# DCDmllm/AnyEdit

Hardware: AMD Instinct MI355X
Metric: edited-images/sec @512x512, 50 DDIM steps (higher is better)
Workload: dtype bf16; 1 GPU; configs[1]: AnySD (SD-1.5 UNet in=8 + task embedding/expert adapters) 512x512 bf16, 50 DDIM steps, batch=4/GPU, 3-branch CFG (UNet batch 12); images_per_gpu=4, ddim_steps=50, cfg_branches=3, hip_graph=True, parallelism=dp1 (image-sharded, no data-path collective)

## Files before the change

anyedit_amd/_lib.py:

```python
import ctypes
import os

import torch

_HERE = os.path.dirname(os.path.abspath(__file__))
LIB_PATH = os.environ.get("AE_LIB_PATH") or os.path.join(_HERE, "libanyedit_hip.so")

c_void_p, c_int, c_long, c_float = ctypes.c_void_p, ctypes.c_int, ctypes.c_long, ctypes.c_float

SIGNATURES = {
    "ae_version": [],
    "ae_last_error": [],
    "ae_device_arch": [ctypes.c_char_p, c_int],
    "ae_device_info": [ctypes.POINTER(c_int), ctypes.POINTER(c_long), ctypes.POINTER(c_int)],
    "ae_gemm_bf16": [c_void_p, c_long, c_void_p, c_long, c_int, c_void_p, c_long, c_void_p, c_long, c_int, c_int, c_int,
                     c_void_p, c_void_p, c_long, c_void_p, c_long, c_int, c_int, c_int, c_void_p, c_void_p],
    "ae_conv3x3_workspace_floats": [c_int, c_int, c_int, c_int, c_int, c_int, c_int],
    "ae_conv3x3_partials_bf16": [c_void_p, c_void_p, c_int, c_int, c_int, c_int, c_int, c_void_p, c_int, c_void_p, c_void_p],
    "ae_groupnorm_splitk_supported": [c_int, c_int, c_int, c_int, c_int],
    "ae_groupnorm_splitk_nhwc_bf16": [c_void_p, c_int, c_void_p, c_void_p, c_long, c_void_p, c_void_p, c_void_p, c_int, c_int, c_int, c_int, c_float, c_int, c_void_p],
    "ae_conv3x3_bf16": [c_void_p, c_void_p, c_void_p, c_void_p, c_long, c_void_p, c_void_p, c_int, c_int, c_int, c_int, c_int,
                        c_int, c_int, c_int, c_void_p, c_void_p, c_int, c_void_p],
    "ae_conv3x3_up2_bf16": [c_void_p, c_void_p, c_void_p, c_void_p, c_int, c_int, c_int, c_int, c_int, c_void_p, c_void_p],
    "ae_groupnorm_rows_per_chunk": [c_int, c_int],
# ... 16 lines not shown
    "ae_add_bf16": [c_void_p, c_void_p, c_void_p, c_long, c_void_p],
    "ae_axpy_bf16": [c_void_p, c_void_p, c_float, c_void_p, c_long, c_void_p],
    "ae_geglu_fwd_bf16": [c_void_p, c_void_p, c_long, c_int, c_void_p],
    "ae_geglu_bwd_bf16": [c_void_p, c_void_p, c_void_p, c_long, c_int, c_void_p],
    "ae_sumpool2x2_bf16": [c_void_p, c_void_p, c_int, c_int, c_int, c_int, c_void_p],
    "ae_colsum_bf16_f32": [c_void_p, c_void_p, c_int, c_int, c_long, c_void_p],
    "ae_mse_grad_f32": [c_void_p, c_void_p, c_void_p, c_long, c_float, c_void_p],
    "ae_adamw_f32": [c_void_p, c_void_p, c_void_p, c_void_p, c_long, c_float, c_float, c_float, c_float, c_float, c_int, c_float,
                     c_void_p],
    "ae_rowsum_f32": [c_void_p, c_void_p, c_int, c_long, c_void_p],
    "ae_scatter_add_rows_f32": [c_void_p, c_void_p, c_void_p, c_int, c_int, c_int, c_void_p],
    "ae_attn_fp8_workspace_bytes": [c_int, c_int, c_int, c_int, c_int],
    "ae_attn_fwd_fp8": [c_void_p, c_void_p, c_void_p, c_void_p, c_int, c_int, c_int, c_int, c_int] + [c_long] * 12 +
                       [c_float, c_void_p, c_void_p, c_int, c_int, c_void_p, c_long, c_void_p],
    "ae_ln_gemm_supported": [c_int, c_int, c_int, c_int],
    "ae_ln_gemm_bf16": [c_void_p, c_long, c_void_p, c_long, c_void_p, c_long, c_int, c_int, c_int, c_void_p, c_void_p, c_long, c_void_p, c_void_p,
                        c_float, c_int, c_void_p, c_void_p],
    "ae_gemm_ln_plan": [c_int, c_int, c_int, c_int, c_int],
    "ae_xattn_fused_supported": [c_int, c_int, c_int, c_int, c_int, c_int, c_int],
    "ae_xattn_fused_covers": [c_int, c_int, c_int, c_int, c_int, c_int, c_int],
    "ae_xattn_fused_kv_bytes": [],
    "ae_xattn_fused_bf16": [c_void_p, c_long, c_void_p, c_void_p, c_float, c_void_p, c_void_p, c_void_p, c_void_p, c_void_p, c_void_p, c_long, c_int, c_int, c_int, c_int,
                            c_float, c_void_p],
    "ae_ff_fused_supported": [c_int, c_int, c_int],
    "ae_ff_fused_bf16": [c_void_p, c_long, c_void_p, c_void_p, c_float, c_void_p, c_long, c_void_p, c_void_p, c_void_p, c_void_p, c_long,
                         c_void_p, c_long, c_void_p, c_void_p, c_long, c_void_p, c_void_p, c_long, c_int, c_int, c_int, c_void_p],
    "ae_gemm_ln_bf16": [c_void_p, c_long, c_void_p, c_long, c_void_p, c_long, c_int, c_int, c_int, c_void_p, c_void_p, c_long, c_int, c_void_p,
                        c_void_p, c_int, c_void_p, c_float, c_void_p],
    "ae_task_gate_bwd": [c_void_p, c_void_p, c_void_p, c_void_p, c_int, c_int, c_int, c_void_p, c_void_p],
    "ae_task_gate_wgrad": [c_void_p, c_void_p, c_void_p, c_void_p, c_void_p, c_int, c_int, c_int, c_int, c_void_p, c_void_p, c_void_p],
    "ae_expert_kv_fwd": [c_void_p, c_void_p, c_void_p, c_void_p, c_int, c_int, c_int, c_int, c_int, c_void_p],
    "ae_expert_kv_dgrad_slices": [c_int],
    "ae_expert_kv_dgrad": [c_void_p, c_void_p, c_void_p, c_void_p, c_int, c_int, c_int, c_int, c_int, c_void_p, c_void_p],
    "ae_expert_kv_wgrad": [c_void_p, c_void_p, c_void_p, c_void_p, c_int, c_int, c_int, c_int, c_int, c_void_p],
    "ae_transpose_last2": [c_void_p, c_void_p, c_int, c_int, c_int, c_int, c_int, c_int, c_void_p],
    "ae_concat_channels_bf16": [c_void_p, c_int, c_void_p, c_int, c_void_p, c_long, c_void_p],
    "ae_im2col3x3_c8_bf16": [c_void_p, c_void_p, c_int, c_int, c_int, c_void_p],
    "ae_split_channels_bf16": [c_void_p, c_int, c_int, c_void_p, c_void_p, c_long, c_int, c_int, c_void_p],
    "ae_timestep_embedding": [c_void_p, c_void_p, c_void_p, c_void_p, c_int, c_int, c_float, c_void_p],
    "ae_ddim_step_f32": [c_void_p, c_void_p, c_void_p, c_void_p, c_void_p, c_void_p, c_long, c_int, c_float, c_float, c_float,
                         c_float, c_float, c_float, c_float, c_float, c_void_p],
    "ae_ddim_encode_step_f32": [c_void_p, c_void_p, c_void_p, c_long, c_int, c_float, c_float, c_float, c_void_p],
    "ae_plms_combine_f32": [c_void_p, c_void_p, c_void_p, c_void_p, c_void_p, c_long, c_int, c_void_p],
    "ae_mask_blend_f32": [c_void_p, c_void_p, c_void_p, c_void_p, c_void_p, c_int, c_int, c_int, c_float, c_float, c_int, c_void_p],
    "ae_q_sample_f32": [c_void_p, c_void_p, c_void_p, c_void_p, c_void_p, c_int, c_long, c_void_p],
    "ae_silu_to_bf16": [c_void_p, c_int, c_void_p, c_long, c_void_p],
# ... 69 lines not shown
```

anyedit_amd/anysd/model.py:

```python
import torch
import torch.nn as nn

from anyedit_amd import ops
from anyedit_amd.cldm.model import trusted_torch_load
from anyedit_amd.ldm.modules.attention import BasicTransformerBlock

BF16 = torch.bfloat16

EDIT_TYPES = ["add", "remove", "replace", "color_alter", "appearance_alter", "material_alter", "action_change",
              "textual_change", "background_change", "tone_transfer", "style_change", "movement", "outpaint", "rotation_change",
              "resize", "implicit_change", "relation_change", "counting", "visual_reference", "visual_bbox", "visual_depth",
              "visual_scribble", "visual_segment", "visual_sketch", "visual_material_transfer"]


class ImageProjModel(nn.Module):

    def __init__(self, clip_dim=1280, cross_dim=768, tokens=4):
        super().__init__()
        self.tokens, self.cross_dim = tokens, cross_dim
        self.proj = nn.Linear(clip_dim, tokens * cross_dim)
        self.norm = nn.LayerNorm(cross_dim)

    def rows(self, ref_embeds):
        B = ref_embeds.shape[0]
# ... 34 lines not shown
    @torch.no_grad()
    def prepare_conditioning(self, encoder_hidden_states, ref_embeds, edit_code, ip_scale=None):
        B, L, Dc = encoder_hidden_states.shape
        dev = encoder_hidden_states.device
        te = self.task_embs.detach()[edit_code.long()]
        ctx = torch.cat([encoder_hidden_states.float(), te[:, None, :].float()], dim=1)
        context_rows = ctx.reshape(B * (L + 1), Dc).to(BF16).contiguous()
        probs, top1, top1p = self.route(edit_code)
        gate = top1p if ip_scale is None else top1p * ip_scale
        ip_rows = self.image_proj_model.rows(ref_embeds)
        T_ip = self.image_proj_model.tokens
        kv_cache = {}
        for blk, W in zip(self._blocks, self.adapter_modules):
            attn = blk.attn2
            kv_cache[id(attn)] = attn.project_kv(context_rows)
            Wm = W.detach()
            if Wm.dtype != torch.float32 or not Wm.is_contiguous():
                Wm = Wm.float().contiguous()
            kv_ip = ops.expert_kv(ip_rows, Wm, top1, T_ip)
            kv_cache[("adapter", id(attn))] = (kv_ip, gate.float().contiguous())
            img = attn.fused_kv_images(kv_cache[id(attn)], kv_cache[("adapter", id(attn))], B)
            if img is not None:
                kv_cache[("xattn_img", id(attn))] = img
        return context_rows, kv_cache

    @torch.no_grad()
    def denoise(self, x, timesteps, context_rows, kv_cache, emb_pack=None):
        return self.unet.forward_rows(x, timesteps, context_rows, kv_cache=kv_cache, emb_pack=emb_pack)

    def forward(self, noisy_latents, timesteps, encoder_hidden_states, image_embeds, edit_code):
        context_rows, kv_cache = self.prepare_conditioning(encoder_hidden_states, image_embeds, edit_code)
        return self.denoise(noisy_latents, timesteps, context_rows, kv_cache)
```

anyedit_amd/build.py:

```python
import hashlib
import os
import shutil
import subprocess
import sys

HERE = os.path.dirname(os.path.abspath(__file__))
CSRC = os.path.join(HERE, "csrc")
LIB = os.path.join(HERE, "libanyedit_hip.so")
SOURCES = ["c_api.hip", "gemm_conv.hip", "gemm_rowpanel.hip", "ff_fused.hip", "xattn_fused.hip", "attention.hip", "attention_fast.hip", "attention_fp8.hip", "attention_bwd.hip", "norm.hip", "elementwise.hip", "backward.hip", "gate.hip", "expert_kv.hip", "msda.hip",
           "sam_decoder.hip", "clip_text.hip"]
EXTRA = {"gemm_conv.hip": ["-fno-slp-vectorize"], "gemm_rowpanel.hip": ["-fno-slp-vectorize"], "ff_fused.hip": ["-fno-slp-vectorize"], "xattn_fused.hip": ["-fno-slp-vectorize"], "attention.hip": ["-ffinite-math-only"],
         "attention_fast.hip": ["-ffinite-math-only", "-fno-slp-vectorize"], "attention_fp8.hip": ["-ffinite-math-only"],
         "attention_bwd.hip": ["-ffinite-math-only"], "clip_text.hip": ["-ffinite-math-only"]}
FLAGS = ["--offload-arch=gfx950", "-O3", "-std=c++17", "-fPIC", "-fno-gpu-rdc", "-Wno-unused-result"]


def _hipcc():
    for c in (shutil.which("hipcc"), "/opt/rocm/bin/hipcc"):
        if c and os.path.exists(c):
            return c
    raise RuntimeError("hipcc not found: the HIP extension cannot be built")


def _digest():
    h = hashlib.sha256()
    for name in sorted(os.listdir(CSRC)):
        with open(os.path.join(CSRC, name), "rb") as f:
            h.update(name.encode() + f.read())
    h.update((" ".join(FLAGS) + repr(sorted(EXTRA.items()))).encode())
    return h.hexdigest()


def build_library(force=False, verbose=True, variant=None, extra_flags=None):
    lib = LIB if variant is None else os.path.join(HERE, f"libanyedit_hip_{variant}.so")
    extra = {k: list(v) for k, v in EXTRA.items()}
# ... 47 lines not shown
```

anyedit_amd/ldm/modules/attention.py:

```python
import os

import torch
import torch.nn as nn

from anyedit_amd import ops
from anyedit_amd.ldm.util import default, exists
from anyedit_amd.ldm.modules.diffusionmodules.util import Linear, Conv2d, LayerNorm, checkpoint

BF16 = torch.bfloat16
_XATTN_FUSED = os.environ.get("AE_XATTN_FUSED", "0") != "0"
_FF_TAIL = os.environ.get("AE_FF_TAIL", "1") != "0"
_SEG2_160 = os.environ.get("AE_ATTN_SEG2_160", "1") != "0"


def zero_module(module):
    for p in module.parameters():
        p.detach().zero_()
    return module


class _GN6(nn.GroupNorm):

    def _affine(self):
        if ops.cache_stale(self, "_pk", self.weight, self.bias):
# ... 133 lines not shown
                pk["qkv"] = torch.cat([wq, wk, wv], 0).contiguous()
            self._pk = pk
        return self._pk

    def _packed_x(self):
        if ops.cache_stale(self, "_pkx", self.to_q.weight, self.to_out[0].weight, self.to_out[0].bias):
            bo = self.to_out[0].bias
            self._pkx = (ops.pack_xattn_wq(self.to_q.weight), ops.pack_xattn_wo(self.to_out[0].weight), None if bo is None else bo.detach().float().contiguous())
        return self._pkx

    def fused_kv_images(self, kv, adapter, B):
        if not _XATTN_FUSED or self.is_self or self.heads != 8 or self.dim_head != 40 or self.to_q.weight.shape[1] != 320:
            return None
        Nk = kv.shape[0] // B
        T = 0 if adapter is None else adapter[0].shape[0] // B
        if not (64 < Nk <= 80 and T <= 16):
            return None
        return ops.pack_xattn_kv(kv, None if adapter is None else adapter[0], B, Nk, T)

    def project_kv(self, ctx_rows):
        return ops.gemm(ctx_rows, self._packed()["kv"])

    def rows(self, x, B, N, context_rows=None, Nk=None, kv=None, key_mask=None, residual=None, adapter=None, norm=None, rowstats=None,
             out_rowstats=None, kv_img=None):
        h, d = self.heads, self.dim_head
        inner = h * d
        if kv_img is not None and kv is not None and norm is not None and residual is x and key_mask is None and out_rowstats is None:
            Nk_ = kv.shape[0] // B
            T_ = 0 if adapter is None else adapter[0].shape[0] // B
            if ops.xattn_fused_ok(x.shape[0], x.shape[1], h, d, N, Nk_, T_):
                wq_img, wo_img, bo = self._packed_x()
                g_, be_ = norm._affine()
                return ops.xattn_fused(x, g_, be_, norm.eps, wq_img, kv_img, None if adapter is None else adapter[1], wo_img, bo, N, Nk_, T_, self.scale)
        pk = self._packed()

        def proj(wname):
            if norm is None:
                return ops.gemm(x, pk[wname])
            if rowstats is not None and ops.ln_fold_plan(x.shape[0], pk[wname].shape[0], x.shape[1], ops.EPI_NONE, 2):
                wq, s, c = self._packed_ln(wname, norm)
                return ops.gemm_ln(x, rowstats, wq, s, c, norm.eps)
            g, be = norm._affine()
            return ops.ln_gemm(x, g, be, norm.eps, pk[wname])

        if context_rows is None and kv is None:
            qkv = proj("qkv")
            s = (N * 3 * inner, d, 3 * inner)
            o = ops.attention(qkv, qkv[:, inner:], qkv[:, 2 * inner:], B, h, N, N, d, self.scale, s, s, s, key_mask=key_mask)
        else:
            q = proj("q")
            if kv is None:
                kv = self.project_kv(context_rows)
            Nk = kv.shape[0] // B
            qs = (N * inner, d, inner)
            ks = (Nk * 2 * inner, d, 2 * inner)
            if adapter is not None and (d <= 96 or (d == 160 and _SEG2_160)) and key_mask is None:
                kv_ip, gate = adapter
                T_ip = kv_ip.shape[0] // B
                ks_ip = (T_ip * 2 * inner, d, 2 * inner)
                seg2 = (kv_ip, kv_ip[:, inner:], T_ip, ks_ip, ks_ip, gate)
                o = ops.attention(q, kv, kv[:, inner:], B, h, N, Nk, d, self.scale, qs, ks, ks, seg2=seg2)
            else:
                o = ops.attention(q, kv, kv[:, inner:], B, h, N, Nk, d, self.scale, qs, ks, ks, key_mask=key_mask)
                if adapter is not None:
                    kv_ip, gate = adapter
                    T_ip = kv_ip.shape[0] // B
                    ks_ip = (T_ip * 2 * inner, d, 2 * inner)
                    ops.attention(q, kv_ip, kv_ip[:, inner:], B, h, N, T_ip, d, self.scale, qs, ks_ip, ks_ip, out=o,
                                  out_scale=gate, accumulate=True)
        return self.to_out[0].rows(o.reshape(B * N, inner), residual=residual, rowstats=out_rowstats)

    def forward(self, x, context=None, mask=None):
        B, N, C = x.shape
        xr = x.reshape(B * N, C).to(BF16).contiguous()
        ctx = None
        if context is not None:
            ctx = context.reshape(-1, context.shape[-1]).to(BF16).contiguous()
        km = None
        if exists(mask):
# ... 59 lines not shown
        M, C = x.shape
        f1, f2, f3 = self._fold_plan(M, C)
        kv2, adapter, kv_img = None, None, None
        if kv_cache is not None and context_rows is not None and not (ops._TAPE is not None and ops._TAPE.active):
            kv_img = kv_cache.get(("xattn_img", id(self.attn2)))
        use_x = kv_img is not None and not f3 and ops.xattn_fused_ok(M, C, self.attn2.heads, self.attn2.dim_head, N, 78, 0)
        st2 = ops.rowstats_buffer(M, C, x.device) if (f2 and not use_x) else None
        st3 = ops.rowstats_buffer(M, C, x.device) if f3 else None
        x = self.attn1.rows(x, B, N, context_rows=c1, residual=x, norm=self.norm1, rowstats=rowstats if f1 else None, out_rowstats=st2)
        if kv_cache is not None and context_rows is not None:
            key = id(self.attn2)
            kv2 = kv_cache.get(key)
            if kv2 is None:
                kv2 = self.attn2.project_kv(context_rows)
                if not (ops._TAPE is not None and ops._TAPE.active):
                    kv_cache[key] = kv2
            adapter = kv_cache.get(("adapter", key))
            if callable(adapter):
                adapter = adapter()
            if kv_img is None and not f3 and not (ops._TAPE is not None and ops._TAPE.active):
                img = self.attn2.fused_kv_images(kv2, adapter, B)
                if img is not None:
                    kv_cache[("xattn_img", key)] = img
        x = self.attn2.rows(x, B, N, context_rows=context_rows, kv=kv2, residual=x, adapter=adapter, norm=self.norm2, rowstats=st2, out_rowstats=st3,
                            kv_img=kv_img if use_x else None)
        x = self.ff.rows(x, residual=x, norm=self.norm3, rowstats=st3, tail=tail)
        return x

    def forward(self, x, context=None):
        B, N, C = x.shape
        ctx = None if context is None else context.reshape(-1, context.shape[-1]).to(BF16).contiguous()
        y = self.rows(x.reshape(B * N, C).to(BF16).contiguous(), B, N, context_rows=ctx)
        return y.reshape(B, N, C).to(x.dtype)

    _forward = forward


class SpatialTransformer(nn.Module):

    def __init__(self, in_channels, n_heads, d_head, depth=1, dropout=0., context_dim=None, disable_self_attn=False,
                 use_linear=False, use_checkpoint=True):
        super().__init__()
        if exists(context_dim) and not isinstance(context_dim, list):
            context_dim = [context_dim] * depth
        if context_dim is None:
            context_dim = [None] * depth
        self.in_channels = in_channels
        inner_dim = n_heads * d_head
# ... 46 lines not shown
```

anyedit_amd/ops.py:

```python
import torch

import ctypes
import os
import threading

from ._lib import lib, check as _check

BF16 = torch.bfloat16
EPI_NONE, EPI_GELU, EPI_GEGLU, EPI_SILU, EPI_RELU = 0, 1, 2, 3, 4


def _s():
    return torch.cuda.current_stream().cuda_stream


def _p(t):
    return None if t is None else t.data_ptr()


_live = threading.local()


def _tmp(t):
    if t is not None:
# ... 281 lines not shown
    _chk(wo_img, BF16, "xattn_fused.wo_img", 3)
    _chk(kv_img, BF16, "xattn_fused.kv_img", 3)
    _chk(gamma, torch.float32, "xattn_fused.gamma", 1)
    _chk(beta, torch.float32, "xattn_fused.beta", 1)
    M, C = x.shape
    B = M // rows_per_sample
    if tuple(wq_img.shape) != (8, 48, 320) or tuple(wo_img.shape) != (4, 320, 112) or tuple(kv_img.shape) != (B, 8, 14848) or not (wq_img.is_contiguous() and wo_img.is_contiguous()
                                                                                                                                    and kv_img.is_contiguous()) or x.stride(1) != 1:
        raise ValueError(f"xattn_fused: x {tuple(x.shape)}, images {tuple(wq_img.shape)} / {tuple(wo_img.shape)} / {tuple(kv_img.shape)} do not fit together")
    if gate is not None:
        _chk(gate, torch.float32, "xattn_fused.gate", 1)
        if gate.numel() != B:
            raise ValueError("xattn_fused: one gate per sample")
    if bo is not None:
        _chk(bo, torch.float32, "xattn_fused.bo", 1)
    if out is None:
        out = torch.empty(M, C, dtype=BF16, device=x.device)
    _chk(out, BF16, "xattn_fused.out", 2)
    check(lib.ae_xattn_fused_bf16(_p(x), x.stride(0), _p(gamma), _p(beta), float(eps), _p(wq_img), _p(kv_img), _p(gate), _p(wo_img), _p(bo), _p(out), out.stride(0), M,
                                  rows_per_sample, Nk, T, float(scale), _s()), "ae_xattn_fused_bf16")
    return out


def colstats_buffer(M, N, device):
    return torch.empty((M + 31) // 32, N, 2, dtype=torch.float32, device=device)


_GN_COLSTATS = os.environ.get("AE_GN_COLSTATS", "1") != "0"


def want_colstats(HW):
    return _GN_COLSTATS and HW > 256 and HW % 32 == 0 and not (_TAPE is not None and _TAPE.active)


def gemm(a, w, bias=None, residual=None, addvec=None, rows_per_batch=0, epilogue=EPI_NONE, out_f32=False, a2=None, out=None, colstats=None,
         rowstats=None):
    if rowstats is not None:
        if _TAPE is not None and _TAPE.active:
            raise ValueError("gemm: row statistics are not recorded on the training tape (ln_fold_plan is False while it records)")
        if addvec is not None or a2 is not None or out_f32 or colstats is not None or epilogue != EPI_NONE:
            raise ValueError("gemm: rowstats goes with a plain bf16 GEMM (+bias, +residual) only")
        return _gemm_ln(a, w, bias, residual, EPI_NONE, out, rowstats, None, None, 0.0)
    if _TAPE is not None and _TAPE.active:
        return _TAPE.gemm(a, w, bias=bias, residual=residual, addvec=addvec, rows_per_batch=rows_per_batch, epilogue=epilogue, out_f32=out_f32, a2=a2, out=out)
    _chk(a, BF16, "gemm.a", 2)
    _chk(w, BF16, "gemm.w", 2)
# ... 1232 lines not shown
    nb = 2 * (x.numel() + 16 * Cin * Cout) + 2 * y.numel()
    return f"gemm_kernel<{tl},conv3x3,up2x2>|M={y.shape[0]} Cin={Cin} Cout={Cout}", 2.0 * y.shape[0] * Cout * 4 * Cin, float(nb)


conv3x3_up2 = _wrap_profiled(conv3x3_up2, _up2_label)
xattn_fused = _wrap_profiled(xattn_fused, lambda _r, x, gamma, beta, eps, wq_img, kv_img, gate, wo_img, bo, rows_per_sample, Nk, T, scale, out=None: (
    f"xattn_fused_kernel<C=320>|M={x.shape[0]} Nk={Nk}+{T}", 2.0 * x.shape[0] * 320 * (2 * 320 + 2 * (Nk + T)), float(2 * (3 * x.numel() + wq_img.numel() + wo_img.numel() + kv_img.numel()))))
ff_fused = _wrap_profiled(ff_fused, lambda _r, x, gamma, beta, eps, w1, b1, w2img, b2, residual=None, out=None, w3=None, b3=None, residual3=None, colstats=None: (
    f"ff_fused_kernel<C=320{',proj_out' if w3 is not None else ''}>|M={x.shape[0]} H={w1.shape[0] // 2}",
    2.0 * x.shape[0] * x.shape[1] * (3 * (w1.shape[0] // 2) + (x.shape[1] if w3 is not None else 0)),
    float(2 * (x.numel() * (2 + (residual is not None and residual is not x) + (residual3 is not None)) + w1.numel() + w2img.numel() + (w3.numel() if w3 is not None else 0))),
    2 if colstats is not None else 1))
_ln_gemm_fused = _wrap_profiled(_ln_gemm_launch, _ln_gemm_label)
_gemm_ln_launch = _wrap_profiled(_gemm_ln_launch, _gemm_ln_label)
gemm = _wrap_profiled(gemm, _gemm_label)
attention_fp8 = _wrap_profiled(attention_fp8, _attn8_label)
conv3x3 = _wrap_profiled(conv3x3, _conv_label)
conv3x3_partials = _wrap_profiled(conv3x3_partials, lambda _r, x, w, B, H, W, k_order=0: (
    f"gemm_kernel<{_tile_label(x.shape[0], w.shape[0], True, 9 * (-(-x.shape[1] // 64) * 64), False, x.shape[1] % 64 == 0)},conv3x3>|M={x.shape[0]} Cin={x.shape[1]} Cout={w.shape[0]} s1 partials",
    2.0 * x.shape[0] * w.shape[0] * 9 * x.shape[1], float(2 * (x.numel() + 9 * x.shape[1] * w.shape[0]) + 2 * x.shape[0] * w.shape[0]), 1))
groupnorm_splitk = _wrap_profiled(groupnorm_splitk, lambda _r, partials, *a, **k: (
    f"groupnorm(splitK fold)|rows={_r.shape[0]} C={_r.shape[1]}", 0.0, 2.0 * _r.numel() * 2, 1))
attention = _wrap_profiled(attention, _attn_label)
groupnorm = _wrap_profiled(groupnorm, _gn_label)
layernorm = _wrap_profiled(layernorm, _ln_label)
expert_kv = _wrap_profiled(expert_kv, lambda _r, x, W, experts, tokens: (
    f"expert_kv_fwd_kernel|rows={x.shape[0]} N={W.shape[1]} Dc={W.shape[2]}", 2.0 * x.shape[0] * W.shape[1] * W.shape[2], 4.0 * (x.shape[0] // tokens) * W.shape[1] * W.shape[2]))
expert_kv_dgrad = _wrap_profiled(expert_kv_dgrad, lambda _r, dy, W, experts, tokens: (
    f"expert_kv_dgrad_kernel|rows={dy.shape[0]} N={W.shape[1]} Dc={W.shape[2]}", 2.0 * dy.shape[0] * W.shape[1] * W.shape[2], 4.0 * (dy.shape[0] // tokens) * W.shape[1] * W.shape[2]))
expert_kv_wgrad = _wrap_profiled(expert_kv_wgrad, lambda _r, dy, x, experts, tokens, n_experts, out=None: (
    f"expert_kv_wgrad_kernel|rows={dy.shape[0]} N={dy.shape[1]} Dc={x.shape[1]} E={n_experts}", 2.0 * dy.shape[0] * dy.shape[1] * x.shape[1], 4.0 * n_experts * dy.shape[1] * x.shape[1]))
```

include/anyedit_hip.h:

```cpp
#ifndef ANYEDIT_HIP_H
#define ANYEDIT_HIP_H

#ifdef __cplusplus
extern "C" {
#endif

#define AE_OK 0
#define AE_ERR_ARG (-1)
#define AE_ERR_LAUNCH (-2)
#define AE_ERR_UNSUPPORTED (-3)

#define AE_EPI_NONE 0
#define AE_EPI_GELU 1
#define AE_EPI_GEGLU 2
#define AE_EPI_SILU 3
#define AE_EPI_RELU 4

int ae_version(void);
const char* ae_last_error(void);
int ae_device_arch(char* buf, int n);
int ae_device_info(int* cus, long* hbm_bytes, int* clock_khz);

int ae_gemm_bf16(const void* A, long lda, const void* A2, long lda2, int Ksplit, const void* W, long ldw, void* C, long ldc,
                 int M, int N, int K, const float* bias, const void* residual, long ldr, const float* addvec, long addvec_ld,
                 int rows_per_batch, int epilogue, int out_f32, float* colstats, void* stream);

int ae_ln_gemm_supported(int M, int N, int K, int epilogue);
int ae_ln_gemm_bf16(const void* A, long lda, const void* W, long ldw, void* C, long ldc, int M, int N, int K, const float* bias,
                    const void* residual, long ldr, const float* ln_gamma, const float* ln_beta, float ln_eps, int epilogue,
                    float* colstats , void* stream);

int ae_gemm_ln_plan(int M, int N, int K, int epilogue, int mode);
int ae_gemm_ln_bf16(const void* A, long lda, const void* W, long ldw, void* C, long ldc, int M, int N, int K, const float* bias,
                    const void* residual, long ldr, int epilogue, float* rowstats_out, const float* ln_stats, int ln_parts,
                    const float* ln_colsum, float ln_eps, void* stream);

int ae_ff_fused_supported(int M, int C, int H);
int ae_ff_fused_bf16(const void* X, long ldx, const float* ln_gamma, const float* ln_beta, float ln_eps, const void* W1, long ldw1, const float* b1,
                     const void* W2img, const float* b2, const void* residual, long ldr, const void* W3, long ldw3, const float* b3,
                     const void* residual3, long ldr3, float* colstats, void* Y, long ldy, int M, int C, int H, void* stream);

int ae_xattn_fused_supported(int M, int C, int heads, int head_dim, int rows_per_sample, int Nk, int T);
int ae_xattn_fused_covers(int M, int C, int heads, int head_dim, int rows_per_sample, int Nk, int T);
long ae_xattn_fused_kv_bytes(void);
int ae_xattn_fused_bf16(const void* X, long ldx, const float* ln_gamma, const float* ln_beta, float ln_eps, const void* Wq_img, const void* KV_img, const float* gate,
                        const void* Wo_img, const float* bo, void* Y, long ldy, int M, int rows_per_sample, int Nk, int T, float scale, void* stream);

long ae_conv3x3_workspace_floats(int B, int H, int W, int Cin, int Cout, int stride, int upsample2x);
int ae_conv3x3_partials_bf16(const void* x, const void* w, int B, int H, int W, int Cin, int Cout, float* workspace, int k_order, int* splitk_out, void* stream);
int ae_conv3x3_bf16(const void* x, const void* w, const float* bias, const float* addvec, long addvec_ld, const void* residual,
                    void* y, int B, int H, int W, int Cin, int Cout, int stride, int upsample2x, int out_f32, float* workspace,
                    float* colstats , int k_order, void* stream);

int ae_conv3x3_up2_bf16(const void* x, const void* w4, const float* bias, void* y, int B, int H, int W, int Cin, int Cout,
                        float* colstats, void* stream);

int ae_groupnorm_rows_per_chunk(int HW, int C);
long ae_groupnorm_workspace_floats(int B, int HW, int C, int groups);
int ae_groupnorm_splitk_supported(int B, int HW, int C, int groups, int splitk);
int ae_groupnorm_splitk_nhwc_bf16(const float* partial, int splitk, const float* bias, const float* addvec, long addvec_ld, const float* gamma, const float* beta,
                                  void* y, int B, int HW, int C, int groups, float eps, int act, void* stream);
 * colstats / colstats2: optional per-channel slab statistics of x / x2 as written by the kernels that PRODUCED them (the `colstats`
 * output of ae_gemm_bf16 / ae_ln_gemm_bf16 / ae_conv3x3_bf16: [B*HW/32][C1][2] and [B*HW/32][C-C1][2]; HW % 32 == 0).  With them the
 * statistics pass over the activation is skipped: one block per (sample, group) folds the slab sums, then the apply launch runs.    */
int ae_groupnorm_nhwc_bf16(const void* x, const void* x2, int C1, const float* gamma, const float* beta, void* y, int B, int HW,
                           int C, int groups, float eps, int act, float* workspace, int* counters, float* stat_out,
                           const float* colstats, const float* colstats2, void* stream);

int ae_layernorm_bf16(const void* x, const float* gamma, const float* beta, void* y, int M, int C, float eps, void* stream);
// ... 126 lines not shown
```

Measured before the change: 6.420 edited-images/sec.

## Add dedicated cross-attention kernel with precomputed per-head K/V LDS image

Adds a specialized cross-attention kernel for the UNet's short context (text keys plus expert IP tokens, up to 96 slots). A per-step prep kernel packs K and V for each (batch, head) into a contiguous image that is DMA'd straight into LDS. The kernel then does QK^T and PV with MFMA in a single pass and uses two softmax groups blended by the gate, replacing the generic segmented attention path. This targets the overhead of the general flash-attention path on tiny key counts, at the cost of an extra image buffer and a narrow shape envelope.

Measured after the change: 6.461 edited-images/sec (median of 6 runs). No clear change (+0.6%).

```diff
diff --git a/anyedit_amd/_lib.py b/anyedit_amd/_lib.py
--- a/anyedit_amd/_lib.py
+++ b/anyedit_amd/_lib.py
@@ -62,6 +62,9 @@
     "ae_xattn_fused_kv_bytes": [],
     "ae_xattn_fused_bf16": [c_void_p, c_long, c_void_p, c_void_p, c_float, c_void_p, c_void_p, c_void_p, c_void_p, c_void_p, c_void_p, c_long, c_int, c_int, c_int, c_int,
                             c_float, c_void_p],
+    "ae_ctx_attn_supported": [c_int, c_int, c_int, c_int, c_int, c_int, c_long, c_long],
+    "ae_ctx_kv_image_bf16": [c_void_p, c_void_p, c_void_p, c_int, c_int, c_int, c_int, c_int, c_void_p],
+    "ae_ctx_attn_bf16": [c_void_p, c_long, c_void_p, c_void_p, c_void_p, c_long, c_int, c_int, c_int, c_int, c_int, c_int, c_float, c_void_p],
     "ae_ff_fused_supported": [c_int, c_int, c_int],
     "ae_ff_fused_bf16": [c_void_p, c_long, c_void_p, c_void_p, c_float, c_void_p, c_long, c_void_p, c_void_p, c_void_p, c_void_p, c_long,
                          c_void_p, c_long, c_void_p, c_void_p, c_long, c_void_p, c_void_p, c_long, c_int, c_int, c_int, c_void_p],
diff --git a/anyedit_amd/anysd/model.py b/anyedit_amd/anysd/model.py
--- a/anyedit_amd/anysd/model.py
+++ b/anyedit_amd/anysd/model.py
@@ -80,6 +80,9 @@
             img = attn.fused_kv_images(kv_cache[id(attn)], kv_cache[("adapter", id(attn))], B)
             if img is not None:
                 kv_cache[("xattn_img", id(attn))] = img
+            Nk = L + 1
+            if ops.ctx_attn_ok(B, attn.heads, attn.dim_head, 1, Nk, T_ip):
+                kv_cache[("ctx_img", id(attn))] = ops.ctx_kv_image(kv_cache[id(attn)], kv_ip, B, attn.heads, attn.dim_head, Nk, T_ip)
         return context_rows, kv_cache
 
     @torch.no_grad()
diff --git a/anyedit_amd/build.py b/anyedit_amd/build.py
--- a/anyedit_amd/build.py
+++ b/anyedit_amd/build.py
@@ -7,10 +7,10 @@
 HERE = os.path.dirname(os.path.abspath(__file__))
 CSRC = os.path.join(HERE, "csrc")
 LIB = os.path.join(HERE, "libanyedit_hip.so")
-SOURCES = ["c_api.hip", "gemm_conv.hip", "gemm_rowpanel.hip", "ff_fused.hip", "xattn_fused.hip", "attention.hip", "attention_fast.hip", "attention_fp8.hip", "attention_bwd.hip", "norm.hip", "elementwise.hip", "backward.hip", "gate.hip", "expert_kv.hip", "msda.hip",
+SOURCES = ["c_api.hip", "gemm_conv.hip", "gemm_rowpanel.hip", "ff_fused.hip", "xattn_fused.hip", "attention.hip", "attention_fast.hip", "attention_ctx.hip", "attention_fp8.hip", "attention_bwd.hip", "norm.hip", "elementwise.hip", "backward.hip", "gate.hip", "expert_kv.hip", "msda.hip",
            "sam_decoder.hip", "clip_text.hip"]
 EXTRA = {"gemm_conv.hip": ["-fno-slp-vectorize"], "gemm_rowpanel.hip": ["-fno-slp-vectorize"], "ff_fused.hip": ["-fno-slp-vectorize"], "xattn_fused.hip": ["-fno-slp-vectorize"], "attention.hip": ["-ffinite-math-only"],
-         "attention_fast.hip": ["-ffinite-math-only", "-fno-slp-vectorize"], "attention_fp8.hip": ["-ffinite-math-only"],
+         "attention_fast.hip": ["-ffinite-math-only", "-fno-slp-vectorize"], "attention_ctx.hip": ["-ffinite-math-only", "-fno-slp-vectorize"], "attention_fp8.hip": ["-ffinite-math-only"],
          "attention_bwd.hip": ["-ffinite-math-only"], "clip_text.hip": ["-ffinite-math-only"]}
 FLAGS = ["--offload-arch=gfx950", "-O3", "-std=c++17", "-fPIC", "-fno-gpu-rdc", "-Wno-unused-result"]
 
diff --git a/anyedit_amd/csrc/attention_ctx.hip b/anyedit_amd/csrc/attention_ctx.hip
--- /dev/null
+++ b/anyedit_amd/csrc/attention_ctx.hip
@@ -0,0 +1,366 @@
+#include "common.hpp"
+#include <stdlib.h>
+#include <type_traits>
+
+namespace {
+
+typedef __attribute__((ext_vector_type(16))) float f32x16;
+typedef __attribute__((ext_vector_type(4))) short s16x4v;
+
+constexpr int CTX_SLOTS = 96;
+constexpr float CLOG2E = 1.4426950408889634f;
+constexpr float CMASKED = -1.0e30f;
+
+struct CtxArgs {
+    const bf16_t* q; const bf16_t* img; const float* gate; bf16_t* o;
+    long q_ld, o_ld;
+    int B, H, Nq, Nk, T, ng;
+    float scale;
+};
+
+__device__ __forceinline__ void ctx_dma_wait_and_barrier() {
+#if defined(__HIP_DEVICE_COMPILE__)
+    asm volatile("s_waitcnt vmcnt(0) lgkmcnt(0)" ::: "memory");
+    __builtin_amdgcn_s_barrier();
+    asm volatile("" ::: "memory");
+#endif
+}
+
+__device__ __forceinline__ s16x4v ctx_lds_tr16(const char* p) {
+#if defined(__HIP_DEVICE_COMPILE__)
+    return __builtin_amdgcn_ds_read_tr16_b64_v4i16((__attribute__((address_space(3))) s16x4v*)p);
+#else
+    return s16x4v{};
+#endif
+}
+
+__device__ __forceinline__ float sum_bf16x2(uint32_t w, float den) {
+#if defined(__HIP_DEVICE_COMPILE__) && __has_builtin(__builtin_amdgcn_fdot2_f32_bf16)
+    union { uint32_t u; bf16x2_t b; } a, one;
+    a.u = w;
+    one.u = 0x3F803F80u;
+    return __builtin_amdgcn_fdot2_f32_bf16(a.b, one.b, den, false);
+#else
+    return den + bf16lo(w) + bf16hi(w);
+#endif
+}
+
+template <int D, int OCC, int NFT>
+__global__ __launch_bounds__(256, OCC) void ctx_attn_kernel(const CtxArgs p) {
+    static_assert(D == 40 || D == 80 || D == 160, "head dims of the UNet's cross-attention layers");
+    constexpr int KS = (D + 15) / 16;
+    constexpr bool QPAD = (D % 16) != 0;
+    constexpr int NDB = (D + 31) / 32;
+    constexpr int NFULL = D / 32, REM = D % 32, RS = 2 * REM;
+    constexpr int ROWB = 2 * D;
+    constexpr int KB = CTX_SLOTS * ROWB;
+    constexpr int IMGB = 2 * KB;
+    constexpr int ZERO_OFF = IMGB;
+    constexpr int LDSB = IMGB + 128;
+    constexpr int NPIECE = IMGB / 1024;
+    static_assert(IMGB % 1024 == 0, "whole 1-KiB DMA pieces");
+    constexpr int MAXP = (NPIECE + 3) / 4;
+    constexpr int NKK = CTX_SLOTS / 16;
+    static_assert(NFT >= 0 && NFT <= NKK, "text-only K steps");
+    constexpr bool G0 = NFT < NKK, G1 = NFT + 1 < NKK;
+    constexpr int NBLK = (NFT + 1 < NKK ? NFT + 1 : NKK - 1) / 2 + 1;
+
+    __shared__ __attribute__((aligned(16))) char smem[LDSB];
+
+    const int tid = threadIdx.x, lane = tid & 63;
+    const int wave = __builtin_amdgcn_readfirstlane(tid >> 6);
+    const int l31 = lane & 31, hi = lane >> 5, l15 = lane & 15, g = lane >> 4;
+    const int nqb = (p.Nq + 128 * p.ng - 1) / (128 * p.ng);
+    const int vb = xcd_remap(blockIdx.x, nqb * p.B * p.H);
+    const int bh = vb / nqb, qb = vb - bh * nqb;
+    const int b = bh / p.H, h = bh - b * p.H;
+    int q0 = qb * 128 * p.ng + wave * 32;
+    const int nk = p.Nk, nt = p.Nk + p.T;
+
+    const int lds0 = (int)(uintptr_t)((__attribute__((address_space(3))) char*)smem);
+    {
+        const __amdgpu_buffer_rsrc_t rs = __builtin_amdgcn_make_buffer_rsrc(const_cast<bf16_t*>(p.img) + (long)bh * (IMGB / 2), 0, IMGB, 0x00020000);
+#pragma unroll
+        for (int i = 0; i < MAXP; ++i) {
+            const int j = wave + 4 * i;
+            if (j < NPIECE) ae_dma16(rs, lds0 + j * 1024, j * 1024 + lane * 16);
+        }
+    }
+    if (tid < 8) *reinterpret_cast<u32x4*>(smem + ZERO_OFF + tid * 16) = (u32x4){0u, 0u, 0u, 0u};
+
+    const bf16_t* qp = p.q + (long)b * p.Nq * p.q_ld + (long)h * D;
+    constexpr bool PREF = D < 160;
+    u32x4 qf[KS], qn[PREF ? KS : 1];
+    auto load_q = [&](auto& dst, int qbase) {
+        const int qrow = min(qbase + l31, p.Nq - 1);
+#pragma unroll
+        for (int ks = 0; ks < KS; ++ks) {
+            const int d0 = 16 * ks + 8 * hi;
+            dst[ks] = *reinterpret_cast<const u32x4*>(qp + (long)qrow * p.q_ld + (d0 < D ? d0 : 0));
+        }
+    };
+    load_q(qf, q0);
+
+    const int kaddr = l31 * ROWB + hi * 16;
+    const int klast = (QPAD && hi) ? ZERO_OFF : kaddr + (KS - 1) * 32;
+    const int klast_step = (QPAD && hi) ? 0 : 32 * ROWB;
+    const int vrow = 4 * hi + (l15 >> 2);
+    const int vcolb = (16 * (g & 1) + 4 * (l15 & 3)) * 2;
+    const int vfull = KB + vrow * 64 + vcolb;
+    const int vrem = KB + NFULL * CTX_SLOTS * 64 + vrow * RS + vcolb;
+
+    const float c = p.scale * CLOG2E;
+    const float gate = p.gate ? p.gate[b] : 1.0f;
+    const int ta = nk - 16 * NFT, eb0 = min(max(nt - 16 * NFT, 0), 16), eb1 = min(max(nt - 16 * (NFT + 1), 0), 16);
+    bf16_t* op = p.o + (long)b * p.Nq * p.o_ld + (long)h * D;
+
+    u32x4 srcring[2];
+    auto retire_src = [&](u32x4 frag, f32x16& acc) __attribute__((always_inline)) {
+        asm volatile("" : "+v"(acc) : "v"(srcring[0]));
+        srcring[0] = srcring[1];
+        srcring[1] = frag;
+    };
+
+    ctx_dma_wait_and_barrier();
+
+    for (int gi = 0; gi < p.ng; ++gi) {
+        if (gi) {
+            q0 += 128;
+            if (q0 - wave * 32 >= p.Nq) break;
+            if (PREF) {
+#pragma unroll
+                for (int ks = 0; ks < KS; ++ks) qf[ks] = qn[ks];
+            } else load_q(qf, q0);
+        }
+        if (PREF && gi + 1 < p.ng) load_q(qn, q0 + 128);
+        if (QPAD && hi) qf[KS - 1] = (u32x4){0u, 0u, 0u, 0u};
+        srcring[0] = srcring[1] = qf[0];
+
+        f32x16 s[NBLK];
+#pragma unroll
+        for (int blk = 0; blk < NBLK; ++blk) {
+#pragma unroll
+            for (int r = 0; r < 16; ++r) s[blk][r] = 0.f;
+#pragma unroll
+            for (int ks = 0; ks < KS; ++ks) {
+                const int ka = (ks == KS - 1) ? klast + blk * klast_step : kaddr + blk * 32 * ROWB + ks * 32;
+                const u32x4 kf = *reinterpret_cast<const u32x4*>(smem + ka);
+                s[blk] = __builtin_amdgcn_mfma_f32_32x32x16_bf16(as_bf16x8(kf), as_bf16x8(qf[ks]), s[blk], 0, 0, 0);
+                retire_src(kf, s[blk]);
+            }
+        }
+
+        float m1 = CMASKED, m2 = CMASKED;
+#pragma unroll
+        for (int kk = 0; kk < NFT; ++kk)
+#pragma unroll
+            for (int e = 0; e < 8; ++e) m1 = fmaxf(m1, s[kk >> 1][8 * (kk & 1) + e]);
+        float t1[8], t2[2][8];
+#pragma unroll
+        for (int e = 0; e < 8; ++e) {
+            const int off = 4 * hi + (e & 3) + 8 * (e >> 2);
+            t1[e] = t2[0][e] = t2[1][e] = CMASKED;
+            if constexpr (G0) {
+                const float v = s[NFT >> 1][8 * (NFT & 1) + e];
+                t1[e] = off < ta ? v : CMASKED;
+                t2[0][e] = (off >= ta && off < eb0) ? v : CMASKED;
+            }
+            if constexpr (G1) t2[1][e] = off < eb1 ? s[(NFT + 1) >> 1][8 * ((NFT + 1) & 1) + e] : CMASKED;
+            m1 = fmaxf(m1, t1[e]);
+            m2 = fmaxf(m2, fmaxf(t2[0][e], t2[1][e]));
+        }
+        if constexpr (KS == 3) asm volatile("" : "+v"(m1), "+v"(m2) : "v"(qf[0]), "v"(qf[1]), "v"(qf[2]), "v"(srcring[0]), "v"(srcring[1]));
+        else if constexpr (KS == 5) asm volatile("" : "+v"(m1), "+v"(m2) : "v"(qf[0]), "v"(qf[1]), "v"(qf[2]), "v"(qf[3]), "v"(qf[4]), "v"(srcring[0]), "v"(srcring[1]));
+        else asm volatile("" : "+v"(m1), "+v"(m2) : "v"(qf[0]), "v"(qf[1]), "v"(qf[2]), "v"(qf[3]), "v"(qf[4]), "v"(qf[5]), "v"(qf[6]), "v"(qf[7]), "v"(qf[8]), "v"(qf[9]),
+                          "v"(srcring[0]), "v"(srcring[1]));
+        m1 = fmaxf(m1, __shfl_xor(m1, 32, 64));
+        m2 = fmaxf(fmaxf(m2, __shfl_xor(m2, 32, 64)), -1.0e20f);
+        const float m1c = m1 * c, m2c = m2 * c;
+
+        uint32_t pk[NFT > 0 ? NFT : 1][4], pt[4] = {0u, 0u, 0u, 0u}, pe[2][4] = {{0u, 0u, 0u, 0u}, {0u, 0u, 0u, 0u}};
+        float den1 = 0.f, den2 = 0.f;
+#pragma unroll
+        for (int kk = 0; kk < NFT; ++kk)
+#pragma unroll
+            for (int i = 0; i < 4; ++i) {
+                const int blk = kk >> 1, r = 8 * (kk & 1) + 2 * i;
+                pk[kk][i] = pack_bf16x2(__builtin_amdgcn_exp2f(__builtin_fmaf(s[blk][r], c, -m1c)), __builtin_amdgcn_exp2f(__builtin_fmaf(s[blk][r + 1], c, -m1c)));
+                den1 = sum_bf16x2(pk[kk][i], den1);
+            }
+        if constexpr (G0) {
+#pragma unroll
+            for (int i = 0; i < 4; ++i) {
+                pt[i] = pack_bf16x2(__builtin_amdgcn_exp2f(__builtin_fmaf(t1[2 * i], c, -m1c)), __builtin_amdgcn_exp2f(__builtin_fmaf(t1[2 * i + 1], c, -m1c)));
+                den1 = sum_bf16x2(pt[i], den1);
+#pragma unroll
+                for (int j = 0; j < (G1 ? 2 : 1); ++j) {
+                    pe[j][i] = pack_bf16x2(__builtin_amdgcn_exp2f(__builtin_fmaf(t2[j][2 * i], c, -m2c)), __builtin_amdgcn_exp2f(__builtin_fmaf(t2[j][2 * i + 1], c, -m2c)));
+                    den2 = sum_bf16x2(pe[j][i], den2);
+                }
+            }
+        }
+        den1 += __shfl_xor(den1, 32, 64);
+        den2 += __shfl_xor(den2, 32, 64);
+        const float inv = 1.0f / den1;
+        const float rho = p.T > 0 ? gate * den1 / (p.T > 0 ? den2 : 1.0f) : 0.f;
+
+        f32x16 o[NDB];
+#pragma unroll
+        for (int db = 0; db < NDB; ++db)
+#pragma unroll
+            for (int r = 0; r < 16; ++r) o[db][r] = 0.f;
+        auto pv_step = [&](int kk, const uint32_t (&pb)[4], auto masked_tag, int lim) __attribute__((always_inline)) {
+            constexpr bool MASK = decltype(masked_tag)::value;
+            const u32x4 pbv = (u32x4){pb[0], pb[1], pb[2], pb[3]};
+            u32x4 vm = {0u, 0u, 0u, 0u};
+            if (MASK) {
+                const int s0 = 4 * hi;
+                vm.x = (s0 + 0 < lim ? 0x0000FFFFu : 0u) | (s0 + 1 < lim ? 0xFFFF0000u : 0u);
+                vm.y = (s0 + 2 < lim ? 0x0000FFFFu : 0u) | (s0 + 3 < lim ? 0xFFFF0000u : 0u);
+                vm.z = (s0 + 8 < lim ? 0x0000FFFFu : 0u) | (s0 + 9 < lim ? 0xFFFF0000u : 0u);
+                vm.w = (s0 + 10 < lim ? 0x0000FFFFu : 0u) | (s0 + 11 < lim ? 0xFFFF0000u : 0u);
+            }
+#pragma unroll
+            for (int db = 0; db < NDB; ++db) {
+                const int va = (db < NFULL) ? vfull + db * (CTX_SLOTS * 64) + kk * (16 * 64) : vrem + kk * (16 * RS);
+                const int vstep = (db < NFULL) ? 8 * 64 : 8 * RS;
+                union { struct { s16x4v a, b; } s; u32x4 u; } vf;
+                vf.s.a = ctx_lds_tr16(smem + va);
+                vf.s.b = ctx_lds_tr16(smem + va + vstep);
+                if (MASK) vf.u &= vm;
+                o[db] = __builtin_amdgcn_mfma_f32_32x32x16_bf16(as_bf16x8(vf.u), as_bf16x8(pbv), o[db], 0, 0, 0);
+                retire_src(vf.u, o[db]);
+            }
+        };
+        if constexpr (G0) {
+            pv_step(NFT, pe[0], std::true_type{}, eb0);
+            if constexpr (G1) pv_step(NFT + 1, pe[1], std::true_type{}, eb1);
+#pragma unroll
+            for (int db = 0; db < NDB; ++db)
+#pragma unroll
+                for (int r = 0; r < 16; ++r) o[db][r] *= rho;
+        }
+#pragma unroll
+        for (int kk = 0; kk < NFT; ++kk) pv_step(kk, pk[kk], std::false_type{}, 16);
+        if constexpr (G0) pv_step(NFT, pt, std::true_type{}, eb0);
+        float first[NDB];
+#pragma unroll
+        for (int db = 0; db < NDB; ++db) first[db] = o[db][0] * inv;
+#pragma unroll
+        for (int db = 0; db < NDB; ++db) asm volatile("" : "+v"(first[db]) : "v"(srcring[0]), "v"(srcring[1]), "v"(pt[0]), "v"(pt[1]), "v"(pt[2]), "v"(pt[3]));
+        asm volatile("" : "+v"(first[0]) : "v"(pe[0][0]), "v"(pe[0][1]), "v"(pe[0][2]), "v"(pe[0][3]), "v"(pe[1][0]), "v"(pe[1][1]), "v"(pe[1][2]), "v"(pe[1][3]));
+#pragma unroll
+        for (int kk = 0; kk < NFT; ++kk)
+#pragma unroll
+            for (int db = 0; db < NDB; ++db) asm volatile("" : "+v"(first[db]) : "v"(pk[kk][0]), "v"(pk[kk][1]), "v"(pk[kk][2]), "v"(pk[kk][3]));
+
+        const int qrow = q0 + l31;
+        if (qrow < p.Nq) {
+#pragma unroll
+            for (int db = 0; db < NDB; ++db)
+#pragma unroll
+                for (int r4 = 0; r4 < 4; ++r4) {
+                    const int d = 32 * db + 8 * r4 + 4 * hi;
+                    if (d < D)
+                        *reinterpret_cast<u32x2*>(op + (long)qrow * p.o_ld + d) =
+                            (u32x2){pack_bf16x2(r4 == 0 ? first[db] : o[db][4 * r4] * inv, o[db][4 * r4 + 1] * inv), pack_bf16x2(o[db][4 * r4 + 2] * inv, o[db][4 * r4 + 3] * inv)};
+                }
+        }
+    }
+}
+
+__global__ __launch_bounds__(256) void ctx_kv_image_kernel(const bf16_t* __restrict__ kv, const bf16_t* __restrict__ kv_ip, bf16_t* __restrict__ img, int B, int H, int D,
+                                                          int Nk, int T, long total) {
+    const long idx = (long)blockIdx.x * 256 + threadIdx.x;
+    if (idx >= total) return;
+    const int cpi = CTX_SLOTS * D / 4;
+    const int bh = (int)(idx / cpi);
+    int e = (int)(idx - (long)bh * cpi) * 8;
+    const int b = bh / H, h = bh - b * H;
+    const int KE = CTX_SLOTS * D, nfull = D / 32, rem = D % 32;
+    const bool isV = e >= KE;
+    int slot, d;
+    if (!isV) { slot = e / D; d = e - slot * D; }
+    else {
+        e -= KE;
+        if (e < nfull * CTX_SLOTS * 32) { const int db = e / (CTX_SLOTS * 32); e -= db * CTX_SLOTS * 32; slot = e >> 5; d = 32 * db + (e & 31); }
+        else { e -= nfull * CTX_SLOTS * 32; slot = e / rem; d = 32 * nfull + (e - slot * rem); }
+    }
+    const long ld = 2L * H * D;
+    const long col = (isV ? (long)H * D : 0) + (long)h * D + d;
+    u32x4 v = {0u, 0u, 0u, 0u};
+    if (slot < Nk) v = *reinterpret_cast<const u32x4*>(kv + ((long)b * Nk + slot) * ld + col);
+    else if (slot < Nk + T) v = *reinterpret_cast<const u32x4*>(kv_ip + ((long)b * T + (slot - Nk)) * ld + col);
+    *reinterpret_cast<u32x4*>(img + idx * 8) = v;
+}
+
+int ctx_cu_count() {
+    static int cus = 0;
+    if (cus == 0) {
+        int dev = 0, n = 0;
+        if (hipGetDevice(&dev) != hipSuccess || hipDeviceGetAttribute(&n, hipDeviceAttributeMultiprocessorCount, dev) != hipSuccess || n <= 0) n = 256;
+        cus = n;
+    }
+    return cus;
+}
+
+template <int D, int OCC>
+int ctx_launch(CtxArgs a, hipStream_t stream) {
+    const long units = (long)a.B * a.H * ((a.Nq + 127) / 128);
+    const long slots = (long)ctx_cu_count() * OCC;
+    int ng = (int)((units + slots - 1) / slots);
+    const char* e = getenv("AE_CTX_NG");
+    if (e && atoi(e) > 0) ng = atoi(e);
+    const int groups = (a.Nq + 127) / 128;
+    if (ng > groups) ng = groups;
+    if (ng < 1) ng = 1;
+    a.ng = ng;
+    const long blocks = (long)a.B * a.H * ((a.Nq + 128 * ng - 1) / (128 * ng));
+    const dim3 grid((unsigned)blocks), block(256);
+    switch (a.Nk >> 4) {
+        case 0: hipLaunchKernelGGL((ctx_attn_kernel<D, OCC, 0>), grid, block, 0, stream, a); break;
+        case 1: hipLaunchKernelGGL((ctx_attn_kernel<D, OCC, 1>), grid, block, 0, stream, a); break;
+        case 2: hipLaunchKernelGGL((ctx_attn_kernel<D, OCC, 2>), grid, block, 0, stream, a); break;
+        case 3: hipLaunchKernelGGL((ctx_attn_kernel<D, OCC, 3>), grid, block, 0, stream, a); break;
+        case 4: hipLaunchKernelGGL((ctx_attn_kernel<D, OCC, 4>), grid, block, 0, stream, a); break;
+        case 5: hipLaunchKernelGGL((ctx_attn_kernel<D, OCC, 5>), grid, block, 0, stream, a); break;
+        default: hipLaunchKernelGGL((ctx_attn_kernel<D, OCC, 6>), grid, block, 0, stream, a); break;
+    }
+    return ae_check_launch("ctx_attn_kernel");
+}
+
+}
+
+extern "C" int ae_ctx_attn_supported(int B, int H, int D, int Nq, int Nk, int T, long q_ld, long o_ld) {
+    if (!(D == 40 || D == 80 || D == 160)) return 0;
+    if (B < 1 || H < 1 || Nq < 1 || Nk < 1 || T < 0 || T > 16 || Nk + T > CTX_SLOTS) return 0;
+    if (q_ld < (long)H * D || o_ld < (long)H * D || q_ld % 8 != 0 || o_ld % 4 != 0) return 0;
+    const long groups = (Nq + 127) / 128;
+    if ((long)B * H * groups > 0x7FFFFFFFL || (long)B * H * (CTX_SLOTS * D / 4) > 0x7FFFFFFFL || (long)B * Nq > 0x7FFFFFFFL) return 0;
+    return 1;
+}
+
+extern "C" int ae_ctx_kv_image_bf16(const void* kv, const void* kv_ip, void* img, int B, int H, int D, int Nk, int T, void* stream) {
+    AE_REQUIRE(kv && img, "ae_ctx_kv_image_bf16: null tensor");
+    AE_REQUIRE(ae_ctx_attn_supported(B, H, D, 1, Nk, T, (long)H * D, (long)H * D), "ae_ctx_kv_image_bf16: B=%d H=%d D=%d Nk=%d T=%d outside the envelope", B, H, D, Nk, T);
+    AE_REQUIRE(T == 0 || kv_ip, "ae_ctx_kv_image_bf16: T=%d expert keys but no expert tensor", T);
+    const long total = (long)B * H * (CTX_SLOTS * D / 4);
+    hipLaunchKernelGGL(ctx_kv_image_kernel, dim3((unsigned)((total + 255) / 256)), dim3(256), 0, (hipStream_t)stream, (const bf16_t*)kv, (const bf16_t*)kv_ip, (bf16_t*)img,
+                       B, H, D, Nk, T, total);
+    return ae_check_launch("ctx_kv_image_kernel");
+}
+
+extern "C" int ae_ctx_attn_bf16(const void* q, long q_ld, const void* img, const float* gate, void* out, long o_ld, int B, int H, int D, int Nq, int Nk, int T, float scale,
+                                void* stream) {
+    AE_REQUIRE(q && img && out, "ae_ctx_attn_bf16: null tensor");
+    AE_REQUIRE(scale > 0.f, "ae_ctx_attn_bf16: scale must be positive");
+    if (!ae_ctx_attn_supported(B, H, D, Nq, Nk, T, q_ld, o_ld)) {
+        ae_set_error("ae_ctx_attn_bf16: B=%d H=%d D=%d Nq=%d Nk=%d T=%d ld=%ld/%ld outside the envelope", B, H, D, Nq, Nk, T, q_ld, o_ld);
+        return AE_ERR_UNSUPPORTED;
+    }
+    CtxArgs a{(const bf16_t*)q, (const bf16_t*)img, gate, (bf16_t*)out, q_ld, o_ld, B, H, Nq, Nk, T, 1, scale};
+    hipStream_t st = (hipStream_t)stream;
+    if (D == 40) return ctx_launch<40, 3>(a, st);
+    if (D == 80) return ctx_launch<80, 2>(a, st);
+    return ctx_launch<160, 2>(a, st);
+}
diff --git a/anyedit_amd/ldm/modules/attention.py b/anyedit_amd/ldm/modules/attention.py
--- a/anyedit_amd/ldm/modules/attention.py
+++ b/anyedit_amd/ldm/modules/attention.py
@@ -179,7 +179,7 @@
         return ops.gemm(ctx_rows, self._packed()["kv"])
 
     def rows(self, x, B, N, context_rows=None, Nk=None, kv=None, key_mask=None, residual=None, adapter=None, norm=None, rowstats=None,
-             out_rowstats=None, kv_img=None):
+             out_rowstats=None, kv_img=None, ctx_img=None):
         h, d = self.heads, self.dim_head
         inner = h * d
         if kv_img is not None and kv is not None and norm is not None and residual is x and key_mask is None and out_rowstats is None:
@@ -211,7 +211,10 @@
             Nk = kv.shape[0] // B
             qs = (N * inner, d, inner)
             ks = (Nk * 2 * inner, d, 2 * inner)
-            if adapter is not None and (d <= 96 or (d == 160 and _SEG2_160)) and key_mask is None:
+            T_ = 0 if adapter is None else adapter[0].shape[0] // B
+            if ctx_img is not None and key_mask is None and ops.ctx_attn_ok(B, h, d, N, Nk, T_, q.stride(0), inner):
+                o = ops.ctx_attn(q, ctx_img, None if adapter is None else adapter[1], B, h, d, N, Nk, T_, self.scale)
+            elif adapter is not None and (d <= 96 or (d == 160 and _SEG2_160)) and key_mask is None:
                 kv_ip, gate = adapter
                 T_ip = kv_ip.shape[0] // B
                 ks_ip = (T_ip * 2 * inner, d, 2 * inner)
@@ -317,8 +320,11 @@
                 img = self.attn2.fused_kv_images(kv2, adapter, B)
                 if img is not None:
                     kv_cache[("xattn_img", key)] = img
+        ctx_img = None
+        if kv2 is not None and kv_cache is not None and not (ops._TAPE is not None and ops._TAPE.active):
+            ctx_img = kv_cache.get(("ctx_img", id(self.attn2)))
         x = self.attn2.rows(x, B, N, context_rows=context_rows, kv=kv2, residual=x, adapter=adapter, norm=self.norm2, rowstats=st2, out_rowstats=st3,
-                            kv_img=kv_img if use_x else None)
+                            kv_img=kv_img if use_x else None, ctx_img=ctx_img)
         x = self.ff.rows(x, residual=x, norm=self.norm3, rowstats=st3, tail=tail)
         return x
 
diff --git a/anyedit_amd/ops.py b/anyedit_amd/ops.py
--- a/anyedit_amd/ops.py
+++ b/anyedit_amd/ops.py
@@ -327,6 +327,55 @@
     return out
 
 
+_CTX_ATTN = os.environ.get("AE_CTX_ATTN", "1") != "0"
+CTX_SLOTS = 96
+
+
+def ctx_attn_ok(B, heads, head_dim, Nq, Nk, T, q_ld=None, o_ld=None):
+    inner = heads * head_dim
+    return _CTX_ATTN and not (_TAPE is not None and _TAPE.active) and \
+        bool(lib.ae_ctx_attn_supported(B, heads, head_dim, Nq, Nk, T, inner if q_ld is None else q_ld, inner if o_ld is None else o_ld))
+
+
+def ctx_kv_image(kv, kv_ip, B, heads, head_dim, Nk, T, out=None):
+    _no_tape("ctx_kv_image")
+    inner = heads * head_dim
+    _chk(kv, BF16, "ctx_kv_image.kv", 2)
+    if tuple(kv.shape) != (B * Nk, 2 * inner) or not kv.is_contiguous():
+        raise ValueError(f"ctx_kv_image: kv {tuple(kv.shape)} is not a contiguous [{B * Nk}, {2 * inner}]")
+    if T > 0:
+        _chk(kv_ip, BF16, "ctx_kv_image.kv_ip", 2)
+        if tuple(kv_ip.shape) != (B * T, 2 * inner) or not kv_ip.is_contiguous():
+            raise ValueError(f"ctx_kv_image: kv_ip {tuple(kv_ip.shape)} is not a contiguous [{B * T}, {2 * inner}]")
+    if out is None:
+        out = torch.empty(B, heads, 2 * CTX_SLOTS * head_dim, dtype=BF16, device=kv.device)
+    _chk(out, BF16, "ctx_kv_image.out", 3)
+    if tuple(out.shape) != (B, heads, 2 * CTX_SLOTS * head_dim) or not out.is_contiguous():
+        raise ValueError(f"ctx_kv_image: out {tuple(out.shape)}")
+    check(lib.ae_ctx_kv_image_bf16(_p(kv), _p(kv_ip) if T > 0 else None, _p(out), B, heads, head_dim, Nk, T, _s()), "ae_ctx_kv_image_bf16")
+    return out
+
+
+def ctx_attn(q, img, gate, B, heads, head_dim, Nq, Nk, T, scale, out=None):
+    _no_tape("ctx_attn")
+    inner = heads * head_dim
+    _chk(q, BF16, "ctx_attn.q", 2)
+    _chk(img, BF16, "ctx_attn.img", 3)
+    if q.shape[0] != B * Nq or q.shape[1] < inner or q.stride(1) != 1 or tuple(img.shape) != (B, heads, 2 * CTX_SLOTS * head_dim) or not img.is_contiguous():
+        raise ValueError(f"ctx_attn: q {tuple(q.shape)} / image {tuple(img.shape)} do not fit B={B} heads={heads} head_dim={head_dim} Nq={Nq}")
+    if gate is not None:
+        _chk(gate, torch.float32, "ctx_attn.gate", 1)
+        if gate.numel() != B or not gate.is_contiguous():
+            raise ValueError("ctx_attn: one gate per sample")
+    if out is None:
+        out = torch.empty(B * Nq, inner, dtype=BF16, device=q.device)
+    _chk(out, BF16, "ctx_attn.out", 2)
+    if out.shape[0] != B * Nq or out.shape[1] < inner or out.stride(1) != 1:
+        raise ValueError(f"ctx_attn: out {tuple(out.shape)}")
+    check(lib.ae_ctx_attn_bf16(_p(q), q.stride(0), _p(img), _p(gate), _p(out), out.stride(0), B, heads, head_dim, Nq, Nk, T, float(scale), _s()), "ae_ctx_attn_bf16")
+    return out
+
+
 def colstats_buffer(M, N, device):
     return torch.empty((M + 31) // 32, N, 2, dtype=torch.float32, device=device)
 
@@ -1605,6 +1654,10 @@
 groupnorm_splitk = _wrap_profiled(groupnorm_splitk, lambda _r, partials, *a, **k: (
     f"groupnorm(splitK fold)|rows={_r.shape[0]} C={_r.shape[1]}", 0.0, 2.0 * _r.numel() * 2, 1))
 attention = _wrap_profiled(attention, _attn_label)
+ctx_attn = _wrap_profiled(ctx_attn, lambda _r, q, img, gate, B, heads, head_dim, Nq, Nk, T, scale, out=None: (
+    f"ctx_attn_kernel<D={head_dim}>|Nq={Nq} Nk={Nk} T={T}", 4.0 * B * heads * Nq * (Nk + T) * head_dim, 2.0 * B * heads * head_dim * (2 * Nq + 2 * CTX_SLOTS)))
+ctx_kv_image = _wrap_profiled(ctx_kv_image, lambda _r, kv, kv_ip, B, heads, head_dim, Nk, T, out=None: (
+    f"ctx_kv_image_kernel<D={head_dim}>|Nk={Nk} T={T}", 0.0, 2.0 * B * heads * head_dim * (2 * CTX_SLOTS + 2 * (Nk + T))))
 groupnorm = _wrap_profiled(groupnorm, _gn_label)
 layernorm = _wrap_profiled(layernorm, _ln_label)
 expert_kv = _wrap_profiled(expert_kv, lambda _r, x, W, experts, tokens: (
diff --git a/include/anyedit_hip.h b/include/anyedit_hip.h
--- a/include/anyedit_hip.h
+++ b/include/anyedit_hip.h
@@ -45,6 +45,11 @@
 long ae_xattn_fused_kv_bytes(void);
 int ae_xattn_fused_bf16(const void* X, long ldx, const float* ln_gamma, const float* ln_beta, float ln_eps, const void* Wq_img, const void* KV_img, const float* gate,
                         const void* Wo_img, const float* bo, void* Y, long ldy, int M, int rows_per_sample, int Nk, int T, float scale, void* stream);
+
+int ae_ctx_attn_supported(int B, int H, int D, int Nq, int Nk, int T, long q_ld, long o_ld);
+int ae_ctx_kv_image_bf16(const void* kv, const void* kv_ip, void* img, int B, int H, int D, int Nk, int T, void* stream);
+int ae_ctx_attn_bf16(const void* q, long q_ld, const void* img, const float* gate, void* out, long o_ld, int B, int H, int D, int Nq, int Nk, int T, float scale,
+                     void* stream);
 
 long ae_conv3x3_workspace_floats(int B, int H, int W, int Cin, int Cout, int stride, int upsample2x);
 int ae_conv3x3_partials_bf16(const void* x, const void* w, int B, int H, int W, int Cin, int Cout, float* workspace, int k_order, int* splitk_out, void* stream);
```
